# KTC-Security-Circle/3d-matching

Hardware: AMD Instinct MI355X
Metric: ICP iterations/sec + RANSAC hypotheses/sec, 100k↔100k pts, 1/2/4/8 GPU (higher is better)
Workload: dtype fp16-split MFMA NN screen + fp32 scan, exact fp64 NN decision, fp64 terms/solve; 1 GPU; cfg1: 100000<->100000 synthetic pair per GPU, 50 point-to-plane ICP iterations, brute-force NN (r=0.12), 1 GPU; ns=100000, nt_per_gpu=100000, parallelism=single, comm=none, comm_ranks=1

## Files before the change

### 3d-matching_amd/csrc/lds_dma.h

```cpp
#pragma once

#include <hip/hip_runtime.h>
#include <stdint.h>

namespace m3d {

__device__ __forceinline__ void lds_dma16(const void* src, void* wave_dst) {
  const uint32_t lds = __builtin_amdgcn_readfirstlane(
      (uint32_t)(uintptr_t)(__attribute__((address_space(3))) void*)wave_dst);
  uint32_t saved;
  asm volatile(
      "s_mov_b32 %0, m0\n\ts_mov_b32 m0, %2\n\ts_nop 0\n\tglobal_load_lds_dwordx4 %1, off\n\t"
      "s_mov_b32 m0, %0"
      : "=&s"(saved)
      : "v"(src), "s"(lds)
      : "memory");
}

__device__ __forceinline__ void lds_dma_wait() { asm volatile("s_waitcnt vmcnt(0)" ::: "memory"); }

}
```

### 3d-matching_amd/csrc/nn_brute.hip

```cpp
#include <algorithm>

#include "lds_dma.h"
#include "m3d_internal.h"
#include "nnkey.h"

#ifndef M3D_NN_BRUTE_PLAN_TU
#define M3D_NN_BRUTE_PLAN_TU 0
#endif
#ifndef M3D_NN_CLOCK
#define M3D_NN_CLOCK 0
#endif
#define M3D_NN_TU_MAIN (!M3D_NN_BRUTE_PLAN_TU)
#define M3D_NN_TU_PLAN_KERNEL (M3D_NN_BRUTE_PLAN_TU ? !M3D_NN_CLOCK : M3D_NN_CLOCK)
#if M3D_NN_TU_MAIN || M3D_NN_TU_PLAN_KERNEL

namespace m3d {

typedef _Float16 half8 __attribute__((ext_vector_type(8)));
typedef float floatx16 __attribute__((ext_vector_type(16)));

constexpr int kMG = 2;
constexpr int kMTile = 256;
constexpr int kTH = 4;
constexpr int kMTilePad = 1024;
constexpr int kMBlock = 512;
constexpr int kMQueries = (kMBlock / 64) * kMG * 32;

__device__ __forceinline__ void split16(float x, _Float16& hi, _Float16& lo) {
  hi = (_Float16)x;
  lo = (_Float16)(x - (float)hi);
}

union H8 {
  uint4 u;
  half8 h;
};

__device__ __forceinline__ uint32_t or16(const floatx16& k) {
  const auto b = [&](int i) { return __float_as_uint(k[i]); };
  const uint32_t o0 = __builtin_amdgcn_bitop3_b32(b(0), b(1), b(2), 0xFE);
  const uint32_t o1 = __builtin_amdgcn_bitop3_b32(b(3), b(4), b(5), 0xFE);
  const uint32_t o2 = __builtin_amdgcn_bitop3_b32(b(6), b(7), b(8), 0xFE);
  const uint32_t o3 = __builtin_amdgcn_bitop3_b32(b(9), b(10), b(11), 0xFE);
  const uint32_t o4 = __builtin_amdgcn_bitop3_b32(b(12), b(13), b(14), 0xFE);
  const uint32_t o5 = __builtin_amdgcn_bitop3_b32(o0, o1, o2, 0xFE);
  const uint32_t o6 = __builtin_amdgcn_bitop3_b32(o3, o4, b(15), 0xFE);
  return o5 | o6;
}

__device__ __forceinline__ void thr_operand(half8& b, float thr0, bool& force) {
  const float extra = 1.05f * ((32.0f * 1.01f * 5.9604645e-08f + 2.3841858e-07f) * fabsf(thr0) +
                               5.9604645e-08f);
  float thr = thr0 + extra;
  force = thr > 32768.0f;
  thr = fminf(fmaxf(thr, -32768.0f), 32768.0f);
  const _Float16 th = (_Float16)thr;
  const _Float16 tl = (_Float16)(thr - (float)th);
  b[3] = -th;
  b[4] = -tl;
}

#if M3D_NN_TU_MAIN
#ifndef M3D_NN_TILE_MORTON
#define M3D_NN_TILE_MORTON 1
#endif
__global__ __launch_bounds__(256) void pack16_sorted_kernel(const float4* __restrict__ sorted,
                                                            const int32_t* __restrict__ perm,
                                                            const float4* __restrict__ xyz32,
                                                            int64_t n, int64_t n_pad, float S,
                                                            uint4* __restrict__ mf16,
                                                            float4* __restrict__ mf32) {
  const int64_t k = (int64_t)blockIdx.x * 256 + threadIdx.x;
  if (k >= n_pad) return;
  H8 a, b;
  a.u = make_uint4(0, 0, 0, 0);
  b.u = make_uint4(0, 0, 0, 0);
  if (k < n) {
    const int32_t idx = __float_as_int(sorted[perm != nullptr ? perm[k] : k].w);
    const float4 t = xyz32[idx];
    _Float16 xh, xl, yh, yl, zh, zl, wh, wl;
    split16(t.x * S, xh, xl);
    split16(t.y * S, yh, yl);
    split16(t.z * S, zh, zl);
    split16(t.w * (S * S), wh, wl);
    a.h = half8{xh, xh, xl, yh, yh, yl, zh, zh};
    b.h = half8{zl, wh, wl, (_Float16)1, (_Float16)1, (_Float16)0, (_Float16)0, (_Float16)0};
    mf32[k] = make_float4(t.x, t.y, t.z, __int_as_float(idx));
  } else {
    b.h[1] = (_Float16)65504.0f;
    b.h[3] = (_Float16)1;
    b.h[4] = (_Float16)1;
    mf32[k] = make_float4(1.0e18f, 1.0e18f, 1.0e18f, __int_as_float(-1));
  }
  mf16[k] = a.u;
  mf16[n_pad + k] = b.u;
}

__global__ __launch_bounds__(kMTile) void tile_box_kernel(const float4* __restrict__ mf32,
                                                          float4* __restrict__ box) {
  const float4 t = mf32[(int64_t)blockIdx.x * kMTile + threadIdx.x];
  const bool real = __float_as_int(t.w) >= 0;
  float v[6] = {real ? t.x : kInf,  real ? t.y : kInf,  real ? t.z : kInf,
                real ? t.x : -kInf, real ? t.y : -kInf, real ? t.z : -kInf};
#pragma unroll
  for (int o = 1; o < 64; o <<= 1)
#pragma unroll
    for (int k = 0; k < 6; ++k) {
      const float w = __shfl_xor(v[k], o);
      v[k] = k < 3 ? fminf(v[k], w) : fmaxf(v[k], w);
    }
  __shared__ float part[kMTile / 64][6];
  if ((threadIdx.x & 63) == 0)
#pragma unroll
    for (int k = 0; k < 6; ++k) part[threadIdx.x >> 6][k] = v[k];
  __syncthreads();
  if (threadIdx.x != 0) return;
#pragma unroll
  for (int w = 1; w < kMTile / 64; ++w)
#pragma unroll
    for (int k = 0; k < 6; ++k) v[k] = k < 3 ? fminf(v[k], part[w][k]) : fmaxf(v[k], part[w][k]);
  box[2 * (int64_t)blockIdx.x] = make_float4(v[0], v[1], v[2], 0.0f);
  box[2 * (int64_t)blockIdx.x + 1] = make_float4(v[3], v[4], v[5], 0.0f);
}

hipError_t build_mfma_tiles(const m3d_cloud* c, Grid* g, TmpArena* ta, hipStream_t st) {
  const int64_t n = c->n;
  const int64_t n_pad = std::max<int64_t>((n + kMTilePad - 1) / kMTilePad * kMTilePad, kMTilePad);
  const int32_t* perm = nullptr;
  hipError_t e = M3D_NN_TILE_MORTON ? grid_morton_perm(g, ta, st, &perm) : hipSuccess;
  if (e != hipSuccess) return e;
  e = block_alloc(reinterpret_cast<void**>(&g->mf16), sizeof(uint4) * 2 * n_pad, st);
  if (e == hipSuccess) e = block_alloc(reinterpret_cast<void**>(&g->mf32), sizeof(float4) * n_pad, st);
  if (e == hipSuccess)
    e = block_alloc(reinterpret_cast<void**>(&g->mfbox), sizeof(float4) * 2 * (n_pad / kMTile), st);
  if (e != hipSuccess) {
    block_release(g->mf16);
    block_release(g->mf32);
    block_release(g->mfbox);
    g->mf16 = nullptr;
    g->mf32 = nullptr;
    g->mfbox = nullptr;
    return e;
  }
  g->mf_npad = n_pad;
  pack16_sorted_kernel<<<(unsigned)((n_pad + 255) / 256), 256, 0, st>>>(
      g->pts, perm, c->xyz32, n, n_pad, (float)c->s16, g->mf16, g->mf32);
  tile_box_kernel<<<(unsigned)(n_pad / kMTile), kMTile, 0, st>>>(g->mf32, g->mfbox);
  return hipGetLastError();
}

#endif

struct SeedArgs {
  const int32_t* prev;
  const float4* tgt;
  int64_t nt;
  int on;
};

__device__ __forceinline__ float4 seed_rec_prev(const SeedArgs& sa, int64_t i, int64_t off) {
  const int64_t j = sa.prev[i];
  float4 r = make_float4(0.0f, 0.0f, 0.0f, __int_as_float(-1));
  if (j >= off && j < off + sa.nt) {
    r = sa.tgt[j - off];
    r.w = __int_as_float((int32_t)j);
  }
  return r;
}

struct NnSlice {
  unsigned x, y, S;
};
struct NnPlan {
  const uint32_t* table;
  uint32_t* cnt;
  int nq, S;
};

__device__ __forceinline__ bool publish_k1(const SeedArgs& sa, unsigned y, uint64_t k1, bool changed) {
  return changed || (sa.on && y == 0 && key_real(k1));
}

__device__ void nn_slice_scan(const float4* __restrict__ src32, int64_t ns, const float4* __restrict__ tgt32,
                              int64_t jb, int64_t je, int64_t off, const IcpState* __restrict__ s,
                              int64_t* __restrict__ keys, uint32_t* __restrict__ near2,
                              const SeedArgs& sa, int64_t q0, unsigned bsx, unsigned bsy) {
  const float* Rt = s->Rt32;
  const float r2_hi = s->r2_hi;
  for (int qs = threadIdx.x; qs < kMQueries; qs += kMBlock) {
    const int64_t slot = q0 + (int64_t)bsx * kMQueries + qs;
    if (slot >= ns) return;
    const int64_t i = slot;
    float qx, qy, qz;
    const float4 p = src32[i];
    xform32(Rt, p, qx, qy, qz);
    const int64_t key = sa.on == 0 ? keys[i]
                                   : seed_key_rec(s, sa.on == 2 ? sa.tgt[i] : seed_rec_prev(sa, i, off), qx, qy, qz);
    uint64_t k1 = key == kKeyNone ? make_key(r2_hi, 0xFFFFFFFFu) : (uint64_t)key;
    float k1d = key_real_d2(k1), n2 = kInf;
    const uint64_t k10 = k1;
    for (int64_t j = jb; j < je; ++j) {
      const float4 t = tgt32[j];
      if (__float_as_int(t.w) < 0) continue;
      const float d2 = d2f(qx, qy, qz, t.x, t.y, t.z);
      if (d2 <= r2_hi) near_push(k1, k1d, n2, make_key(d2, (uint32_t)(off + __float_as_int(t.w))), d2);
    }
    const bool pk = publish_k1(sa, bsy, k1, k1 != k10);
    if (pk || n2 < kInf) near_publish((unsigned long long*)&keys[i], &near2[i], k1, n2, pk);
  }
}

__device__ __forceinline__ void nn_push_rows(const float4 (&t)[16], int64_t off, float qx, float qy, float qz,
                                             float r2_hi, uint64_t& k1, float& k1d, float& n2) {
#pragma unroll
  for (int reg = 0; reg < 16; ++reg) {
    const float d2 = d2f(qx, qy, qz, t[reg].x, t[reg].y, t[reg].z);
    const uint64_t kc = make_key(d2, (uint32_t)(off + __float_as_int(t[reg].w)));
    if (d2 <= r2_hi) near_push(k1, k1d, n2, kc, d2);
  }
}

__device__ __forceinline__ void nn_exact_rows(const float4* __restrict__ rows, int64_t off, int h,
                                              float qx, float qy, float qz, float r2_hi,
                                              uint64_t& k1, float& k1d, float& n2) {
  float4 t[16];
#pragma unroll
  for (int reg = 0; reg < 16; ++reg) t[reg] = rows[(reg & 3) + 8 * (reg >> 2) + 4 * h];
  nn_push_rows(t, off, qx, qy, qz, r2_hi, k1, k1d, n2);
}

__device__ __forceinline__ uint64_t shfl_xor64(uint64_t v, int m) {
  const uint32_t lo = (uint32_t)__shfl_xor((int)(uint32_t)v, m);
  const uint32_t hi = (uint32_t)__shfl_xor((int)(uint32_t)(v >> 32), m);
  return ((uint64_t)hi << 32) | lo;
}

__device__ __forceinline__ uint32_t wave_or32(uint32_t v) {
  int x = (int)v;
  x |= __builtin_amdgcn_mov_dpp(x, 0xB1, 0xF, 0xF, false);
  x |= __builtin_amdgcn_mov_dpp(x, 0x4E, 0xF, 0xF, false);
  x |= xor4_dpp(x);
  x |= __builtin_amdgcn_mov_dpp(x, 0x128, 0xF, 0xF, false);
  return (uint32_t)(__builtin_amdgcn_readlane(x, 0) | __builtin_amdgcn_readlane(x, 16) |
                    __builtin_amdgcn_readlane(x, 32) | __builtin_amdgcn_readlane(x, 48));
}

template <bool kMax>
__device__ __forceinline__ float wave_minmax(float v) {
  const auto mm = [](float a, float b) { return kMax ? fmaxf(a, b) : fminf(a, b); };
  v = mm(v, __int_as_float(__builtin_amdgcn_mov_dpp(__float_as_int(v), 0xB1, 0xF, 0xF, false)));
  v = mm(v, __int_as_float(__builtin_amdgcn_mov_dpp(__float_as_int(v), 0x4E, 0xF, 0xF, false)));
  v = mm(v, __int_as_float(xor4_dpp(__float_as_int(v))));
  v = mm(v, __int_as_float(__builtin_amdgcn_mov_dpp(__float_as_int(v), 0x128, 0xF, 0xF, false)));
  const int x = __float_as_int(v);
  return mm(mm(__int_as_float(__builtin_amdgcn_readlane(x, 0)), __int_as_float(__builtin_amdgcn_readlane(x, 16))),
            mm(__int_as_float(__builtin_amdgcn_readlane(x, 32)), __int_as_float(__builtin_amdgcn_readlane(x, 48))));
}

#ifndef M3D_NN_CULL
#define M3D_NN_CULL 1
#endif
#ifndef M3D_NN_REACH
#define M3D_NN_REACH 1
#endif
#ifndef M3D_NN_ENTRY
#define M3D_NN_ENTRY 1
#endif
#ifndef M3D_NN_SEED_REC
#define M3D_NN_SEED_REC 1
#endif
#ifndef M3D_NN_DEFER_BATCH
#define M3D_NN_DEFER_BATCH 1
#endif
#ifndef M3D_NN_DEFER_FILTER
#define M3D_NN_DEFER_FILTER 1
#endif
#if M3D_NN_CLOCK
constexpr int kClkBlocks = 16384, kClkWords = 8;
__device__ unsigned long long g_nn_clock[kClkWords * kClkBlocks];
#endif
struct QBox {
  float lo[3], hi[3], X;
};
__device__ __forceinline__ bool box_out_of_reach(const QBox& q, const float4& tlo, const float4& thi) {
  const float gx = fmaxf(0.0f, fmaxf(q.lo[0] - thi.x, tlo.x - q.hi[0]));
  const float gy = fmaxf(0.0f, fmaxf(q.lo[1] - thi.y, tlo.y - q.hi[1]));
  const float gz = fmaxf(0.0f, fmaxf(q.lo[2] - thi.z, tlo.z - q.hi[2]));
  return d2f(gx, gy, gz, 0.0f, 0.0f, 0.0f) > q.X;
}
__device__ __forceinline__ bool point_out_of_reach(float qx, float qy, float qz, float X, const float (&lo)[3],
                                                   const float (&hi)[3]) {
  const float gx = fmaxf(0.0f, fmaxf(qx - hi[0], lo[0] - qx));
  const float gy = fmaxf(0.0f, fmaxf(qy - hi[1], lo[1] - qy));
  const float gz = fmaxf(0.0f, fmaxf(qz - hi[2], lo[2] - qz));
  return d2f(gx, gy, gz, 0.0f, 0.0f, 0.0f) > X;
}

constexpr int kTT = kTH * kMTile;
constexpr int kSub = kTT / 32;
constexpr uint64_t kGMask = (kSub == 64) ? ~0ull : ((1ull << kSub) - 1ull);
constexpr int kDefer = 16;
static_assert(kMBlock == 2 * kMTile, "one 16-B operand half per thread per half tile");
static_assert(kSub * kMG <= 64, "hit mask holds every (group, sub-tile)");
static_assert(kSub == 32, "one 32-bit hit record per group and tile");
static_assert(kMBlock / 64 == 8, "eight wave boxes, lanes ^1 ^2 ^4");

struct QState {
  float qx, qy, qz, qq;
  int64_t qi;
  uint64_t k1;
  float k1d, n2;
  half8 bq;
};

__device__ __forceinline__ uint64_t group_mask(uint32_t bits) {
  uint64_t m = 0;
#pragma unroll
  for (int g = 0; g < kMG; ++g)
    if ((bits >> g) & 1u) m |= kGMask << (g * kSub);
  return m;
}

__device__ __forceinline__ float load_query(QState& q, QBox& lq, int64_t slot, int h, float4 p, float4 rec,
                                            int64_t ns, const IcpState* __restrict__ s, const SeedArgs& sa,
                                            const int64_t* __restrict__ keys) {
  const float* Rt = s->Rt32;
  const float r2_hi = s->r2_hi, S = s->mfma_scale;
  const int64_t i = slot < ns ? slot : -1;
  q.qi = i;
  q.n2 = kInf;
  float X = -1.0f;
  if (i >= 0) {
    xform32(Rt, p, q.qx, q.qy, q.qz);
    const int64_t key = sa.on ? seed_key_rec(s, rec, q.qx, q.qy, q.qz) : keys[i];
    q.k1 = key == kKeyNone ? make_key(r2_hi, 0xFFFFFFFFu) : (uint64_t)key;
    X = search_bound(key_d2(q.k1), s->band_e, r2_hi);
    lq.lo[0] = fminf(lq.lo[0], q.qx);
    lq.lo[1] = fminf(lq.lo[1], q.qy);
    lq.lo[2] = fminf(lq.lo[2], q.qz);
    lq.hi[0] = fmaxf(lq.hi[0], q.qx);
    lq.hi[1] = fmaxf(lq.hi[1], q.qy);
    lq.hi[2] = fmaxf(lq.hi[2], q.qz);
    lq.X = fmaxf(lq.X, X);
  } else {
    q.qx = q.qy = q.qz = 0.0f;
    q.k1 = (uint64_t)kKeyNone;
  }
  q.k1d = key_real_d2(q.k1);
  q.qq = fmaf(q.qz, q.qz, fmaf(q.qy, q.qy, q.qx * q.qx));
  _Float16 ah, al, bh, bl, ch, cl;
  split16(-2.0f * S * q.qx, ah, al);
  split16(-2.0f * S * q.qy, bh, bl);
  split16(-2.0f * S * q.qz, ch, cl);
  const _Float16 one = (_Float16)1.0f, zero = (_Float16)0.0f;
  q.bq = h == 0 ? half8{ah, al, ah, bh, bl, bh, ch, cl} : half8{ch, one, one, zero, zero, zero, zero, zero};
  return X;
}

__device__ __forceinline__ bool refresh_threshold(QState& q, int h, float X, float eps, float S2) {
  bool fg;
  half8 bt = q.bq;
  thr_operand(bt, X < 0.0f ? -1.0f : ((X - q.qq) + eps) * S2, fg);
  if (h == 1) q.bq = bt;
  return fg;
}

__device__ __forceinline__ QBox reduce_boxes(const QBox& lq, float4 (&qbox)[kMBlock / 64][2], int lane, int wave) {
  float wlo[3], whi[3];
#pragma unroll
  for (int k = 0; k < 3; ++k) {
    wlo[k] = wave_minmax<false>(lq.lo[k]);
    whi[k] = wave_minmax<true>(lq.hi[k]);
  }
  const float wX = wave_minmax<true>(lq.X);
  if (lane == 0) {
    qbox[wave][0] = make_float4(wlo[0], wlo[1], wlo[2], wX);
    qbox[wave][1] = make_float4(whi[0], whi[1], whi[2], 0.0f);
  }
  __syncthreads();
  float4 lo = qbox[lane & 7][0], hi = qbox[lane & 7][1];
#pragma unroll
  for (int o = 1; o < 8; o <<= 1) {
    const auto x = [&](float v) { return __int_as_float(xor_lane(__float_as_int(v), o, kWave)); };
    lo = make_float4(fminf(lo.x, x(lo.x)), fminf(lo.y, x(lo.y)), fminf(lo.z, x(lo.z)), fmaxf(lo.w, x(lo.w)));
    hi = make_float4(fmaxf(hi.x, x(hi.x)), fmaxf(hi.y, x(hi.y)), fmaxf(hi.z, x(hi.z)), 0.0f);
  }
  const auto u = [](float v) { return __int_as_float(__builtin_amdgcn_readfirstlane(__float_as_int(v))); };
  return QBox{{u(lo.x), u(lo.y), u(lo.z)}, {u(hi.x), u(hi.y), u(hi.z)}, u(lo.w)};
}

struct ReachArgs {
  const QState (&q)[kMG];
  const uint32_t& act;
  float be, r2_hi;
  uint64_t (&slot)[2][kMBlock / 64];
  int wave;
};
struct TileCursor {
  const float4* tbox;
  const float4* wbox;
  QBox bx;
  int lane, ntile, ty;
  int tc;
  uint64_t mb, mw;
  int par = 0;

  __device__ __forceinline__ void cull_round(const ReachArgs& ra) {
    const int tl = tc + (lane >> 2) * ty;
    bool kb = tl < ntile, kw = kb;
    float4 tlo = make_float4(0.0f, 0.0f, 0.0f, 0.0f), thi = tlo;
    if (M3D_NN_CULL && kb) {
      const int64_t hb = (int64_t)tl * kTH + (lane & 3);
      tlo = tbox[2 * hb];
      thi = tbox[2 * hb + 1];
      const float4 l0 = wbox[0], u0 = wbox[1];
      const QBox wq{{l0.x, l0.y, l0.z}, {u0.x, u0.y, u0.z}, l0.w};
      kb = !box_out_of_reach(bx, tlo, thi);
      kw = !box_out_of_reach(wq, tlo, thi);
    }
    mb = __ballot(kb);
    mw = __ballot(kw);
#if M3D_NN_CULL && M3D_NN_REACH
    if (mb == 0) return;
    float X[kMG];
#pragma unroll
    for (int g = 0; g < kMG; ++g)
      X[g] = (ra.act >> g) & 1u ? search_bound(key_d2(ra.q[g].k1), ra.be, ra.r2_hi) : -1.0f;
    uint64_t keep = 0;
    for (uint64_t m = mw; m != 0; m &= m - 1) {
      const int b = __builtin_amdgcn_readfirstlane(__builtin_ctzll(m));
      const auto rl = [&](float v) { return __int_as_float(__builtin_amdgcn_readlane(__float_as_int(v), b)); };
      const float lo[3] = {rl(tlo.x), rl(tlo.y), rl(tlo.z)}, hi[3] = {rl(thi.x), rl(thi.y), rl(thi.z)};
      bool reach = false;
#pragma unroll
      for (int g = 0; g < kMG; ++g)
        reach |= ((ra.act >> g) & 1u) &&
                 !point_out_of_reach(ra.q[g].qx, ra.q[g].qy, ra.q[g].qz, X[g], lo, hi);
      if (__any(reach)) keep |= 1ull << b;
    }
    mw = keep;
    par ^= 1;
    if (lane == 0) ra.slot[par][ra.wave] = mw;
    __syncthreads();
    const uint64_t w = ra.slot[par][lane & 7];
    int wl = (int)(uint32_t)w, wh = (int)(uint32_t)(w >> 32);
#pragma unroll
    for (int o = 1; o < 8; o <<= 1) {
      wl |= xor_lane(wl, o, kWave);
      wh |= xor_lane(wh, o, kWave);
    }
    mb = ((uint64_t)(uint32_t)__builtin_amdgcn_readfirstlane(wh) << 32) |
         (uint32_t)__builtin_amdgcn_readfirstlane(wl);
#endif
  }
  __device__ __forceinline__ void next(int& t, uint32_t& hmask, const ReachArgs& ra) {
    for (;;) {
      if (mb != 0) {
        const int k = __builtin_ctzll(mb) >> 2;
        t = tc + k * ty;
        hmask = (uint32_t)(mw >> (4 * k)) & 15u;
        mb &= ~(15ull << (4 * k));
        return;
      }
      tc += 16 * ty;
      if (tc >= ntile) {
        t = ntile;
        hmask = 0;
        return;
      }
      cull_round(ra);
    }
  }
};

__device__ __forceinline__ void stage_tile(uint4 (&dst)[2][kTT], const uint4* __restrict__ tgt16,
                                           int64_t nt_pad, int t, bool dma) {
#pragma unroll
  for (int u = 0; u < kTH; ++u) {
    const int e = threadIdx.x + u * kMBlock;
    const uint4* src = tgt16 + (e / kTT) * nt_pad + (int64_t)t * kTT + e % kTT;
    if (dma)
      lds_dma16(src, &dst[e / kTT][(e % kTT) & ~63]);
    else
      dst[e / kTT][e % kTT] = *src;
  }
}

__device__ __forceinline__ void sweep_tile(uint32_t (&rec)[kMG], const uint4 (&t16)[2][2][kTT], int buf,
                                           int h, int c, uint32_t hmask, const QState (&q)[kMG],
                                           const floatx16& zacc) {
#pragma unroll
  for (int g = 0; g < kMG; ++g) rec[g] = 0;
  constexpr int kSteps = 8 * kMG;
#pragma unroll
  for (int half = 0; half < kTH; ++half) {
    if (!((hmask >> half) & 1u)) {
#pragma unroll
      for (int g = 0; g < kMG; ++g) rec[g] <<= 8;
      continue;
    }
    H8 av[8];
#pragma unroll
    for (int sub = 0; sub < 8; ++sub) av[sub].u = t16[buf][h][half * kMTile + sub * 32 + c];
    floatx16 kc = __builtin_amdgcn_mfma_f32_32x32x16_f16(av[0].h, q[0].bq, zacc, 0, 0, 0);
#pragma unroll
    for (int t = 0; t < kSteps; ++t) {
      floatx16 kn;
      if (t + 1 < kSteps)
        kn = __builtin_amdgcn_mfma_f32_32x32x16_f16(av[(t + 1) / kMG].h, q[(t + 1) % kMG].bq, zacc, 0, 0, 0);
      __builtin_amdgcn_sched_barrier(0);
      rec[t % kMG] = __builtin_amdgcn_alignbit(rec[t % kMG], or16(kc), 31);
      __builtin_amdgcn_sched_barrier(0);
      if (t + 1 < kSteps) kc = kn;
    }
  }
}

__device__ __forceinline__ uint64_t hit_mask(const uint32_t (&rec)[kMG], uint32_t hmask, uint64_t force64) {
  uint64_t hm = 0;
  uint32_t any = rec[0];
#pragma unroll
  for (int g = 1; g < kMG; ++g) any |= rec[g];
  if (__any(any != 0)) {
#pragma unroll
    for (int g = 0; g < kMG; ++g) hm |= (uint64_t)wave_or32(__builtin_bitreverse32(rec[g])) << (g * kSub);
  }
  uint32_t sm = 0;
#pragma unroll
  for (int half = 0; half < kTH; ++half)
    if ((hmask >> half) & 1u) sm |= 0xFFu << (8 * half);
  uint64_t fm = 0;
#pragma unroll
  for (int g = 0; g < kMG; ++g) fm |= (uint64_t)sm << (g * kSub);
  return hm | (force64 & fm);
}

__device__ __forceinline__ bool nn_exact_subtiles(uint64_t mg, const float4* __restrict__ tile, int64_t off,
                                                  int h, float r2_hi, QState& q) {
  const uint64_t kb = q.k1;
  while (mg != 0) {
    const int sub = __builtin_ctzll(mg);
    mg &= mg - 1;
    nn_exact_rows(tile + sub * 32, off, h, q.qx, q.qy, q.qz, r2_hi, q.k1, q.k1d, q.n2);
    const uint64_t o1 = shfl_xor64(q.k1, 32);
    const float on2 = __shfl_xor(q.n2, 32);
    near_merge(q.k1, q.k1d, q.n2, o1, on2);
  }
  return q.k1 != kb;
}

__device__ __forceinline__ uint32_t nn_defer_hits(const half8& a, const half8& bq, const floatx16& zacc) {
  const floatx16 v = __builtin_amdgcn_mfma_f32_32x32x16_f16(a, bq, zacc, 0, 0, 0);
  uint32_t m = 0;
#pragma unroll
  for (int reg = 15; reg >= 0; --reg) m = __builtin_amdgcn_alignbit(m, __float_as_uint(v[reg]), 31);
  return m;
}
__device__ __forceinline__ void nn_push_hits(uint32_t m, const float4* rows, int64_t off, int h, float qx,
                                             float qy, float qz, float r2_hi, uint64_t& k1, float& k1d,
                                             float& n2) {
  while (m != 0) {
    const int reg = __builtin_ctz(m);
    m &= m - 1;
    const float4 t = rows[(reg & 3) + 8 * (reg >> 2) + 4 * h];
    push_within(k1, k1d, n2, d2f(qx, qy, qz, t.x, t.y, t.z), r2_hi, (uint32_t)(off + __float_as_int(t.w)));
  }
}

template <bool kPlan>
__device__ __forceinline__ void nn_mfma_body(const float4* __restrict__ src32, int64_t ns,
                                             const uint4* __restrict__ tgt16, const float4* __restrict__ tgt32,
                                             const float4* __restrict__ tbox, int64_t nt_pad, int64_t off,
                                             const IcpState* __restrict__ s, int64_t* __restrict__ keys,
                                             uint32_t* __restrict__ near2, const SeedArgs& sa, int64_t q0,
                                             const NnPlan& pl) {
#if M3D_NN_ENTRY
  uint32_t e_tab = kPlanEmpty;
  if (kPlan && pl.table != nullptr) e_tab = pl.table[blockIdx.x];
  int32_t st_done = s->done, st_plan = s->plan_ok, st_mfma = s->mfma_ok;
  asm volatile("" : "+s"(st_done), "+s"(st_plan), "+s"(st_mfma), "+s"(e_tab));
  if (st_done) return;
#else
  if (s->done) return;
#endif
#if M3D_NN_CLOCK
  const unsigned long long clk0 = __builtin_amdgcn_s_memrealtime();
#endif
  NnSlice bs{0u, 0u, 0u};
  if (kPlan && pl.table != nullptr) {
#if M3D_NN_ENTRY
    if (st_plan) {
      const uint32_t e = e_tab;
#else
    if (s->plan_ok) {
      const uint32_t e = pl.table[blockIdx.x];
#endif
      if (e == kPlanEmpty) return;
      bs = NnSlice{plan_x(e), plan_y(e), plan_S(e)};
    } else {
      const unsigned y = blockIdx.x / (unsigned)pl.nq;
      if (y >= (unsigned)pl.S) return;
      bs = NnSlice{blockIdx.x - y * (unsigned)pl.nq, y, (unsigned)pl.S};
    }
  }
#if M3D_NN_ENTRY
  if (!st_mfma) {
#else
  if (!s->mfma_ok) {
#endif
    const int64_t tstep = (int64_t)(kPlan ? bs.S : gridDim.y) * kTT;
    for (int64_t t0 = (int64_t)(kPlan ? bs.y : blockIdx.y) * kTT; t0 < nt_pad; t0 += tstep)
      nn_slice_scan(src32, ns, tgt32, t0, min(nt_pad, t0 + kTT), off, s, keys, near2, sa, q0,
                    kPlan ? bs.x : blockIdx.x, kPlan ? bs.y : blockIdx.y);
    return;
  }
  __shared__ uint4 t16[2][2][kTT];
  __shared__ uint64_t dlist[kMBlock / 64][kDefer];
  __shared__ uint32_t dtile[kMBlock / 64][kDefer];
  __shared__ float4 qbox[kMBlock / 64][2];
  __shared__ uint64_t rslot[2][kMBlock / 64];
#if M3D_NN_CLOCK
  __shared__ uint32_t clk_slow, clk_ticket;
  __shared__ unsigned long long clk_exit;
  if (threadIdx.x == 0) {
    clk_slow = 0;
    clk_ticket = 0;
    clk_exit = 0;
  }
  uint32_t clk_halves = 0;
#endif
  uint32_t kept = 0;
  __shared__ uint32_t slice_xy;
  if (kPlan && threadIdx.x == 0) slice_xy = bs.x | (bs.y << 16);
  const int lane = threadIdx.x & 63, wave = threadIdx.x >> 6;
  const int c = lane & 31, h = lane >> 5;
  const float r2_hi = s->r2_hi, eps = s->screen_eps_m, S = s->mfma_scale, be = s->band_e;
  const float S2 = S * S;

  QState q[kMG];
  uint32_t act = 0;
  uint32_t force = 0;
  uint32_t chg = 0;
  QBox lq{{kInf, kInf, kInf}, {-kInf, -kInf, -kInf}, -1.0f};
  const int64_t slot0 = q0 + (kPlan ? (int64_t)bs.x : (int64_t)blockIdx.x) * kMQueries + wave * kMG * 32 + c;
  float4 qp[kMG], qr[kMG];
#pragma unroll
  for (int g = 0; g < kMG; ++g) {
    const int64_t slot = slot0 + g * 32;
    qp[g] = src32[slot < ns ? slot : 0];
    qr[g] = make_float4(0.0f, 0.0f, 0.0f, 0.0f);
  }
  if (sa.on == 2) {
#pragma unroll
    for (int g = 0; g < kMG; ++g) {
      const int64_t slot = slot0 + g * 32;
      qr[g] = sa.tgt[slot < ns ? slot : 0];
    }
  } else if (sa.on) {
#pragma unroll
    for (int g = 0; g < kMG; ++g) {
      const int64_t slot = slot0 + g * 32;
      qr[g] = seed_rec_prev(sa, slot < ns ? slot : 0, off);
    }
  }
#pragma unroll
  for (int g = 0; g < kMG; ++g) {
    const int64_t slot = slot0 + g * 32;
    const float X = load_query(q[g], lq, slot, h, qp[g], qr[g], ns, s, sa, keys);
    if (q[g].qi >= 0) act |= 1u << g;
    if (__any(refresh_threshold(q[g], h, X, eps, S2))) force |= 1u << g;
  }
  const floatx16 zacc = {0.0f, 0.0f, 0.0f, 0.0f, 0.0f, 0.0f, 0.0f, 0.0f,
                         0.0f, 0.0f, 0.0f, 0.0f, 0.0f, 0.0f, 0.0f, 0.0f};
  uint32_t dfr = 0;
#pragma unroll
  for (int g = 0; g < kMG; ++g)
    if (!((force >> g) & 1u) && __all(q[g].qi < 0 || key_real(q[g].k1))) dfr |= 1u << g;
  int dn = 0;
  uint64_t dmask = group_mask(dfr);
  dmask = ((uint64_t)(uint32_t)__builtin_amdgcn_readfirstlane((int)(dmask >> 32)) << 32) |
          (uint32_t)__builtin_amdgcn_readfirstlane((int)(uint32_t)dmask);

  const QBox bx = reduce_boxes(lq, qbox, lane, wave);
  const int ntile = (int)(nt_pad / kTT);
  const ReachArgs ra{q, act, be, r2_hi, rslot, wave};
  TileCursor cur{tbox, qbox[wave], bx, lane, ntile, (int)(kPlan ? bs.S : gridDim.y), (int)(kPlan ? bs.y : blockIdx.y), 0, 0};
  cur.cull_round(ra);
  int t0, t1;
  uint32_t h0, h1;
  cur.next(t0, h0, ra);
  if (t0 < ntile) stage_tile(t16[0], tgt16, nt_pad, t0, false);
  const uint64_t force64 = group_mask(force);
  __syncthreads();
#if M3D_NN_CLOCK
  const unsigned long long clk1 = __builtin_amdgcn_s_memrealtime();
#endif
  int tog = 0;
  for (; t0 < ntile; t0 = t1, h0 = h1) {
    const int buf = kPlan ? (int)(kept & 1u) : tog;
    const int64_t j0 = (int64_t)t0 * kTT;
    if (kPlan || M3D_NN_CLOCK) ++kept;
#if M3D_NN_CLOCK
    clk_halves += (uint32_t)__builtin_popcount(h0);
#endif
    cur.next(t1, h1, ra);
    if (t1 < ntile) stage_tile(t16[buf ^ 1], tgt16, nt_pad, t1, true);
    uint32_t rec[kMG];
    sweep_tile(rec, t16, buf, h, c, h0, q, zacc);
    uint64_t hm = hit_mask(rec, h0, force64);
    const uint64_t hd = hm & dmask;
    if (hd != 0 && dn < kDefer) {
      if (lane == 0) {
        dlist[wave][dn] = hd;
        dtile[wave][dn] = (uint32_t)j0;
      }
      ++dn;
      hm &= ~hd;
    }
#pragma unroll
    for (int g = 0; g < kMG; ++g) {
      const uint64_t mg = (hm >> (g * kSub)) & kGMask;
      if (mg == 0) continue;
      chg |= (uint32_t)nn_exact_subtiles(mg, tgt32 + j0, off, h, r2_hi, q[g]) << g;
      refresh_threshold(q[g], h, (act >> g) & 1u ? search_bound(key_d2(q[g].k1), be, r2_hi) : -1.0f, eps, S2);
    }
    lds_dma_wait();
    __syncthreads();
    if (!kPlan) tog ^= 1;
  }
#if M3D_NN_CLOCK
  const unsigned long long clk2 = __builtin_amdgcn_s_memrealtime();
  if (lane == 0) atomicMax(&clk_slow, clk_halves);
#endif
#if M3D_NN_DEFER_BATCH
  if (dn > 0) {
#if M3D_NN_DEFER_FILTER
    constexpr int kStash = 8;
#else
    constexpr int kStash = 16;
#endif
    static_assert(kStash * kMG <= 32, "a batch's group flags in one word");
    static_assert(sizeof(t16) >= sizeof(float4) * (kMBlock / 64) * kStash * 32, "a stash per wave");
    float4* const stash = reinterpret_cast<float4*>(&t16[0][0][0]) + wave * (kStash * 32);
    const auto uni = [](uint32_t v) { return (uint32_t)__builtin_amdgcn_readfirstlane((int)v); };
    int e = 0;
    uint64_t ent = dlist[wave][0];
    ent = ((uint64_t)uni((uint32_t)(ent >> 32)) << 32) | uni((uint32_t)ent);
    uint32_t base = uni(dtile[wave][0]);
    const auto subs = [](uint64_t m) {
      uint32_t u = 0;
#pragma unroll
      for (int g = 0; g < kMG; ++g) u |= (uint32_t)(m >> (g * kSub)) & (uint32_t)kGMask;
      return u;
    };
    uint32_t U = subs(ent);
    const auto pop = [&](uint32_t& row0, uint32_t& gs) {
      row0 = 0;
      gs = 0;
      while (U == 0) {
        if (e + 1 >= dn) return;
        ++e;
        ent = dlist[wave][e];
        ent = ((uint64_t)uni((uint32_t)(ent >> 32)) << 32) | uni((uint32_t)ent);
        base = uni(dtile[wave][e]);
        U = subs(ent);
      }
      const int sub = __builtin_ctz(U);
      U &= U - 1;
      row0 = base + (uint32_t)sub * 32u;
#pragma unroll
      for (int g = 0; g < kMG; ++g) gs |= (uint32_t)((ent >> (g * kSub + sub)) & 1u) << g;
    };
    uint64_t kb[kMG];
#pragma unroll
    for (int g = 0; g < kMG; ++g) kb[g] = q[g].k1;
    for (;;) {
      uint32_t gsel = 0;
      float4 ld[kStash / 2];
#if M3D_NN_DEFER_FILTER
      H8 av[kStash];
#endif
#pragma unroll
      for (int k = 0; k < kStash / 2; ++k) {
        uint32_t ra, ga, rb, gb;
        pop(ra, ga);
        pop(rb, gb);
        gsel |= (ga | (gb << kMG)) << (2 * kMG * k);
        ld[k] = make_float4(0.0f, 0.0f, 0.0f, 0.0f);
        if (h == 0 ? ga != 0 : gb != 0) ld[k] = tgt32[(int64_t)(h == 0 ? ra : rb) + c];
#if M3D_NN_DEFER_FILTER
        av[2 * k].u = tgt16[(int64_t)h * nt_pad + ra + c];
        av[2 * k + 1].u = tgt16[(int64_t)h * nt_pad + rb + c];
#endif
      }
#pragma unroll
      for (int k = 0; k < kStash / 2; ++k) stash[(2 * k + h) * 32 + c] = ld[k];
      __builtin_amdgcn_fence(__ATOMIC_RELEASE, "wavefront");
      __builtin_amdgcn_wave_barrier();
      __builtin_amdgcn_fence(__ATOMIC_ACQUIRE, "wavefront");
#if M3D_NN_DEFER_FILTER
#pragma unroll
      for (int sl = 0; sl < kStash; ++sl) {
        const uint32_t gs = (gsel >> (kMG * sl)) & ((1u << kMG) - 1u);
        if (gs == 0) break;
        uint32_t hit[kMG];
#pragma unroll
        for (int g = 0; g < kMG; ++g) hit[g] = (gs >> g) & 1u ? nn_defer_hits(av[sl].h, q[g].bq, zacc) : 0u;
#pragma unroll
        for (int g = 0; g < kMG; ++g)
          if ((gs >> g) & 1u)
            nn_push_hits(hit[g], stash + sl * 32, off, h, q[g].qx, q[g].qy, q[g].qz, r2_hi, q[g].k1, q[g].k1d,
                         q[g].n2);
      }
#else
#pragma unroll 1
      for (int sl = 0; sl < kStash; ++sl) {
        const uint32_t gs = (gsel >> (kMG * sl)) & ((1u << kMG) - 1u);
        if (gs == 0) break;
        float4 t[16];
#pragma unroll
        for (int reg = 0; reg < 16; ++reg) t[reg] = stash[sl * 32 + (reg & 3) + 8 * (reg >> 2) + 4 * h];
#pragma unroll
        for (int g = 0; g < kMG; ++g)
          if ((gs >> g) & 1u) nn_push_rows(t, off, q[g].qx, q[g].qy, q[g].qz, r2_hi, q[g].k1, q[g].k1d, q[g].n2);
      }
#endif
      if (U == 0 && e + 1 >= dn) break;
      __builtin_amdgcn_fence(__ATOMIC_RELEASE, "wavefront");
      __builtin_amdgcn_wave_barrier();
    }
#pragma unroll
    for (int g = 0; g < kMG; ++g) {
      const uint64_t o1 = shfl_xor64(q[g].k1, 32);
      const float on2 = __shfl_xor(q[g].n2, 32);
      near_merge(q[g].k1, q[g].k1d, q[g].n2, o1, on2);
      chg |= (uint32_t)(q[g].k1 != kb[g]) << g;
    }
  }
#else
  for (int e = 0; e < dn; ++e) {
    const uint64_t ent = dlist[wave][e];
    const float4* tile = tgt32 + (int64_t)dtile[wave][e];
#pragma unroll
    for (int g = 0; g < kMG; ++g)
      chg |= (uint32_t)nn_exact_subtiles((ent >> (g * kSub)) & kGMask, tile, off, h, r2_hi, q[g]) << g;
  }
#endif
#if M3D_NN_CLOCK
  const unsigned long long clk2b = __builtin_amdgcn_s_memrealtime();
#endif
  const uint32_t sxy = kPlan ? slice_xy : 0u;
  const int64_t sxl = (int64_t)(sxy & 0xFFFFu);
  const unsigned syl = sxy >> 16;
#define M3D_NN_SX (kPlan ? sxl : (int64_t)blockIdx.x)
#define M3D_NN_SY (kPlan ? syl : blockIdx.y)
#pragma unroll
  for (int g = 0; g < kMG; ++g) {
    if (h != 0 || q[g].qi < 0) continue;
#if (M3D_NN_CULL && M3D_NN_REACH) || M3D_NN_DEFER_BATCH
    int cq = c;
    asm volatile("" : "+v"(cq));
    const int64_t qi = q0 + M3D_NN_SX * kMQueries + (wave * kMG + g) * 32 + cq;
#else
    const int64_t qi = q[g].qi;
#endif
    const bool pk = publish_k1(sa, M3D_NN_SY, q[g].k1, (chg >> g) & 1u);
    if (pk || q[g].n2 < kInf) near_publish((unsigned long long*)&keys[qi], &near2[qi], q[g].k1, q[g].n2, pk);
  }
  if (kPlan && pl.cnt != nullptr && threadIdx.x == 0) atomicAdd(&pl.cnt[M3D_NN_SX], kept);
#if M3D_NN_CLOCK
  {
    const unsigned long long clk3 = __builtin_amdgcn_s_memrealtime();
    const int64_t blk = (int64_t)blockIdx.y * gridDim.x + blockIdx.x;
    if (lane == 0) {
      atomicMax(&clk_exit, clk3);
      if (atomicAdd(&clk_ticket, 1u) == kMBlock / 64 - 1 && blk < kClkBlocks) {
        unsigned long long* rec = g_nn_clock + kClkWords * blk;
        rec[0] = clk0;
        rec[1] = clk1;
        rec[2] = clk2;
        rec[3] = atomicMax(&clk_exit, 0ull);
        rec[4] = kept;
        rec[5] = atomicMax(&clk_slow, 0u);
        rec[6] = (unsigned long long)M3D_NN_SX | ((unsigned long long)M3D_NN_SY << 32) | ((unsigned long long)cur.ty << 48);
        rec[7] = clk2b;
      }
    }
  }
#endif
}

#undef M3D_NN_SX
#undef M3D_NN_SY
#define M3D_NN_KERNEL_ARGS                                                                            \
  const float4 *__restrict__ src32, int64_t ns, const uint4 *__restrict__ tgt16,                      \
      const float4 *__restrict__ tgt32, const float4 *__restrict__ tbox, int64_t nt_pad, int64_t off, \
      const IcpState *__restrict__ s, int64_t *__restrict__ keys, uint32_t *__restrict__ near2, SeedArgs sa, int64_t q0
#if M3D_NN_TU_MAIN
__global__ __launch_bounds__(kMBlock) __attribute__((amdgpu_waves_per_eu(4))) void nn_mfma_kernel(M3D_NN_KERNEL_ARGS) {
  nn_mfma_body<false>(src32, ns, tgt16, tgt32, tbox, nt_pad, off, s, keys, near2, sa, q0, NnPlan{nullptr, nullptr, 0, 0});
}
#endif
hipError_t launch_nn_plan_kernel(unsigned blocks, hipStream_t st, M3D_NN_KERNEL_ARGS, NnPlan pl);
int nn_plan_kernel_blocks_per_cu();
#if M3D_NN_TU_PLAN_KERNEL
__global__ __launch_bounds__(kMBlock) __attribute__((amdgpu_waves_per_eu(4))) void nn_mfma_plan_kernel(
    M3D_NN_KERNEL_ARGS, NnPlan pl) {
  nn_mfma_body<true>(src32, ns, tgt16, tgt32, tbox, nt_pad, off, s, keys, near2, sa, q0, pl);
}
hipError_t launch_nn_plan_kernel(unsigned blocks, hipStream_t st, M3D_NN_KERNEL_ARGS, NnPlan pl) {
  nn_mfma_plan_kernel<<<dim3(blocks), kMBlock, 0, st>>>(src32, ns, tgt16, tgt32, tbox, nt_pad, off, s, keys, near2, sa,
                                                        q0, pl);
  return hipGetLastError();
}
int nn_plan_kernel_blocks_per_cu() {
  int per = 0;
  if (hipOccupancyMaxActiveBlocksPerMultiprocessor(&per, nn_mfma_plan_kernel, kMBlock, 0) != hipSuccess) return 0;
  return per > 0 ? per : 1;
}
#endif
#undef M3D_NN_KERNEL_ARGS
#if M3D_NN_TU_MAIN

static int64_t nn_grid_y(int64_t bx, int64_t ntiles, int64_t slots, bool cull) {
  const auto clamped = [&](int64_t S) { return std::min(std::max<int64_t>(S, 1), ntiles); };
  const int64_t s0 = clamped((2048 + bx - 1) / bx);
  if (slots <= 0 || ntiles <= 1) {
    const int64_t per = (ntiles + s0 - 1) / s0;
    return (ntiles + per - 1) / per;
  }
  if (cull) return clamped(slots / bx);
  int64_t best = s0;
  double best_eff = 0.0;
  for (int64_t S = s0; S <= std::min(2 * s0, ntiles); ++S) {
    const int64_t blocks = bx * S, rounds = (blocks + slots - 1) / slots;
    const double eff = (double)blocks / (double)(rounds * slots);
    if (eff > best_eff + 1e-9) {
      best_eff = eff;
      best = S;
    }
  }
  return best;
}

#if M3D_NN_CLOCK
}
extern "C" int m3d_debug_nn_clock(unsigned long long* out, int n) {
  return hipMemcpyFromSymbol(out, HIP_SYMBOL(m3d::g_nn_clock), sizeof(unsigned long long) * (size_t)n) == hipSuccess ? 0 : -1;
}
namespace m3d {
#endif
static bool icp_nn_uses_mfma(const m3d_icp* s) {
  return s->tgrid != nullptr && s->tgrid->mf16 != nullptr;
}

bool icp_nn_range_ok(const m3d_icp* s) {
  if (s->params.nn_method == M3D_NN_GRID) return s->sgrid != nullptr && s->sgrid->mpts != nullptr;
  return icp_nn_uses_mfma(s);
}

hipError_t launch_icp_nn(const m3d_icp* s, int64_t off, bool self_seed, hipStream_t st, int64_t q0,
                         int64_t q1) {
  const int64_t ns = q1 < 0 ? s->src->n : q1;
  if (ns <= q0 || s->tgt->n == 0) return hipSuccess;
  const Grid* tg = s->tgrid;
  const int64_t tt = (int64_t)kTH * kMTile;
  if (!icp_nn_uses_mfma(s) || tg->mf_npad % tt != 0) return hipErrorInvalidValue;
  const int64_t slots = nn_resident_slots();
  const int64_t bx = (ns - q0 + kMQueries - 1) / kMQueries;
  const int64_t gy = nn_grid_y(bx, tg->mf_npad / tt, slots, M3D_NN_CULL != 0);
  const bool by_rec = M3D_NN_SEED_REC != 0 && self_seed && off == 0 && s->tgt->rec64 != nullptr && s->seed != nullptr;
  const SeedArgs sa{s->corr, by_rec ? s->seed : s->tgt->xyz32, s->tgt->n, by_rec ? 2 : self_seed ? 1 : 0};
  const bool planned = nn_plan_on() && s->nn_qblocks > 0 && q0 == 0 && ns == s->src->n && bx == s->nn_qblocks &&
                       bx * gy <= s->nn_budget;
  if (planned)
    return launch_nn_plan_kernel((unsigned)s->nn_budget, st, s->src->xyz32, ns, tg->mf16, tg->mf32, tg->mfbox,
                                 tg->mf_npad, off, s->state, s->keys, s->near2, sa, q0,
                                 NnPlan{s->nn_table, s->nn_cnt, (int)bx, (int)gy});
  nn_mfma_kernel<<<dim3((unsigned)bx, (unsigned)gy), kMBlock, 0, st>>>(
        s->src->xyz32, ns, tg->mf16, tg->mf32, tg->mfbox, tg->mf_npad, off, s->state, s->keys, s->near2, sa, q0);
  return hipGetLastError();
}

int64_t nn_resident_slots() {
  static const int64_t slots = [] {
    int dev = 0, per = 0;
    hipDeviceProp_t p;
    if (hipGetDevice(&dev) != hipSuccess || hipGetDeviceProperties(&p, dev) != hipSuccess) return (int64_t)0;
    if (hipOccupancyMaxActiveBlocksPerMultiprocessor(&per, nn_mfma_kernel, kMBlock, 0) != hipSuccess)
      return (int64_t)0;
    const int pp = nn_plan_kernel_blocks_per_cu();
    per = per > 0 ? per : 1;
    if (pp > 0 && pp < per) per = pp;
    return (int64_t)p.multiProcessorCount * per;
  }();
  return slots;
}

bool nn_plan_on() {
  static const bool on = [] {
    const char* e = getenv("M3D_NN_PLAN");
    return !(e && atoi(e) == 0);
  }();
  return on;
}

void nn_plan_shape(int64_t ns, int32_t* qblocks, int32_t* budget) {
  const int64_t slots = nn_resident_slots(), bx = (ns + kMQueries - 1) / kMQueries;
  const bool ok = M3D_NN_CULL != 0 && slots > 0 && bx >= 1 && bx < slots && bx <= kPlanMaxQ && slots <= 0xFFFF;
  *qblocks = ok ? (int32_t)bx : 0;
  *budget = ok ? (int32_t)slots : 0;
}

PlanArgs nn_plan_args(const m3d_icp* s) {
  PlanArgs pa;
  if (!nn_plan_on() || s->nn_qblocks <= 0 || s->tgrid == nullptr) return pa;
  pa.cnt = s->nn_cnt;
  pa.seen = s->nn_seen;
  pa.table = s->nn_table;
  pa.n = s->nn_qblocks;
  pa.budget = s->nn_budget;
  pa.cap = (int32_t)plan_cap(kPlanSmax, s->tgrid->mf_npad / ((int64_t)kTH * kMTile));
  return pa;
}

#endif

}
#endif
```

Before: 20550 ICP iter/s (100k src x 100k tgt per GPU).

## Pack surviving tile halves into dense LDS windows and deepen DMA prefetch

```diff
diff --git a/3d-matching_amd/csrc/lds_dma.h b/3d-matching_amd/csrc/lds_dma.h
--- a/3d-matching_amd/csrc/lds_dma.h
+++ b/3d-matching_amd/csrc/lds_dma.h
@@ -19,4 +19,14 @@
 
 __device__ __forceinline__ void lds_dma_wait() { asm volatile("s_waitcnt vmcnt(0)" ::: "memory"); }
 
+__device__ __forceinline__ void lds_dma_wait_older(uint32_t newer) {
+  switch (newer) {
+    case 0: asm volatile("s_waitcnt vmcnt(0)" ::: "memory"); break;
+    case 1: asm volatile("s_waitcnt vmcnt(1)" ::: "memory"); break;
+    case 2: asm volatile("s_waitcnt vmcnt(2)" ::: "memory"); break;
+    case 3: asm volatile("s_waitcnt vmcnt(3)" ::: "memory"); break;
+    default: asm volatile("s_waitcnt vmcnt(4)" ::: "memory"); break;
+  }
 }
+
+}
diff --git a/3d-matching_amd/csrc/nn_brute.hip b/3d-matching_amd/csrc/nn_brute.hip
--- a/3d-matching_amd/csrc/nn_brute.hip
+++ b/3d-matching_amd/csrc/nn_brute.hip
@@ -272,6 +272,9 @@
 #ifndef M3D_NN_DEFER_BATCH
 #define M3D_NN_DEFER_BATCH 1
 #endif
+#ifndef M3D_NN_PACK
+#define M3D_NN_PACK 1
+#endif
 #ifndef M3D_NN_DEFER_FILTER
 #define M3D_NN_DEFER_FILTER 1
 #endif
@@ -404,6 +407,9 @@
   int tc;
   uint64_t mb, mw;
   int par = 0;
+#if M3D_NN_CLOCK
+  uint32_t need = 0;
+#endif
 
   __device__ __forceinline__ void cull_round(const ReachArgs& ra) {
     const int tl = tc + (lane >> 2) * ty;
@@ -459,6 +465,9 @@
         const int k = __builtin_ctzll(mb) >> 2;
         t = tc + k * ty;
         hmask = (uint32_t)(mw >> (4 * k)) & 15u;
+#if M3D_NN_CLOCK
+        need += (uint32_t)__builtin_popcount((uint32_t)(mb >> (4 * k)) & 15u);
+#endif
         mb &= ~(15ull << (4 * k));
         return;
       }
@@ -471,7 +480,42 @@
       cull_round(ra);
     }
   }
+  __device__ __forceinline__ bool next_half(uint32_t& row, uint32_t& mine, uint32_t& kept, const ReachArgs& ra) {
+    for (;;) {
+      if (mb != 0) {
+        const int b = __builtin_ctzll(mb);
+        row = (uint32_t)(tc + (b >> 2) * ty) * (uint32_t)kTT + (uint32_t)(b & 3) * (uint32_t)kMTile;
+        mine = (uint32_t)(mw >> b) & 1u;
+        mb &= mb - 1;
+        if (((mb >> (b & ~3)) & 15ull) == 0) ++kept;
+#if M3D_NN_CLOCK
+        ++need;
+#endif
+        return true;
+      }
+      if (tc >= ntile) return false;
+      tc += 16 * ty;
+      if (tc >= ntile) return false;
+      cull_round(ra);
+    }
+  }
 };
+
+__device__ __forceinline__ uint32_t stage_window(TileCursor& cur, uint4 (&dst)[2][kTT], uint32_t (&wrow)[kTH],
+                                                 const uint4* __restrict__ tgt16, int64_t nt_pad, int wave,
+                                                 uint32_t& kept, const ReachArgs& ra) {
+  uint32_t w = 0;
+#pragma unroll 1
+  for (int n = 0; n < kTH; ++n) {
+    uint32_t row, mine;
+    if (!cur.next_half(row, mine, kept, ra)) break;
+    const uint4* src = tgt16 + ((wave >> 2) ? nt_pad : 0) + row + (threadIdx.x & (kMTile - 1));
+    lds_dma16(src, &dst[wave >> 2][n * kMTile + (wave & 3) * 64]);
+    if (threadIdx.x == 0) wrow[n] = row;
+    w += 0x100u | (mine << n);
+  }
+  return w;
+}
 
 __device__ __forceinline__ void stage_tile(uint4 (&dst)[2][kTT], const uint4* __restrict__ tgt16,
                                            int64_t nt_pad, int t, bool dma) {
@@ -542,6 +586,22 @@
     const int sub = __builtin_ctzll(mg);
     mg &= mg - 1;
     nn_exact_rows(tile + sub * 32, off, h, q.qx, q.qy, q.qz, r2_hi, q.k1, q.k1d, q.n2);
+    const uint64_t o1 = shfl_xor64(q.k1, 32);
+    const float on2 = __shfl_xor(q.n2, 32);
+    near_merge(q.k1, q.k1d, q.n2, o1, on2);
+  }
+  return q.k1 != kb;
+}
+
+__device__ __forceinline__ bool nn_exact_slots(uint64_t mg, const float4* __restrict__ tgt32,
+                                               const uint32_t (&wrow)[kTH], int64_t off, int h, float r2_hi,
+                                               QState& q) {
+  const uint64_t kb = q.k1;
+  while (mg != 0) {
+    const int sub = __builtin_ctzll(mg);
+    mg &= mg - 1;
+    const uint32_t row0 = (uint32_t)__builtin_amdgcn_readfirstlane((int)wrow[sub >> 3]) + (uint32_t)(sub & 7) * 32u;
+    nn_exact_rows(tgt32 + row0, off, h, q.qx, q.qy, q.qz, r2_hi, q.k1, q.k1d, q.n2);
     const uint64_t o1 = shfl_xor64(q.k1, 32);
     const float on2 = __shfl_xor(q.n2, 32);
     near_merge(q.k1, q.k1d, q.n2, o1, on2);
@@ -614,9 +674,11 @@
                     kPlan ? bs.x : blockIdx.x, kPlan ? bs.y : blockIdx.y);
     return;
   }
+  constexpr bool kPack = M3D_NN_PACK == 2 || (M3D_NN_PACK == 1 && !kPlan);
   __shared__ uint4 t16[2][2][kTT];
   __shared__ uint64_t dlist[kMBlock / 64][kDefer];
-  __shared__ uint32_t dtile[kMBlock / 64][kDefer];
+  __shared__ uint32_t dtile[kMBlock / 64][kDefer][kPack ? kTH : 1];
+  __shared__ uint32_t wrow[2][kTH];
   __shared__ float4 qbox[kMBlock / 64][2];
   __shared__ uint64_t rslot[2][kMBlock / 64];
 #if M3D_NN_CLOCK
@@ -686,47 +748,95 @@
   const ReachArgs ra{q, act, be, r2_hi, rslot, wave};
   TileCursor cur{tbox, qbox[wave], bx, lane, ntile, (int)(kPlan ? bs.S : gridDim.y), (int)(kPlan ? bs.y : blockIdx.y), 0, 0};
   cur.cull_round(ra);
-  int t0, t1;
-  uint32_t h0, h1;
-  cur.next(t0, h0, ra);
-  if (t0 < ntile) stage_tile(t16[0], tgt16, nt_pad, t0, false);
-  const uint64_t force64 = group_mask(force);
-  __syncthreads();
-#if M3D_NN_CLOCK
-  const unsigned long long clk1 = __builtin_amdgcn_s_memrealtime();
-#endif
-  int tog = 0;
-  for (; t0 < ntile; t0 = t1, h0 = h1) {
-    const int buf = kPlan ? (int)(kept & 1u) : tog;
-    const int64_t j0 = (int64_t)t0 * kTT;
-    if (kPlan || M3D_NN_CLOCK) ++kept;
-#if M3D_NN_CLOCK
-    clk_halves += (uint32_t)__builtin_popcount(h0);
-#endif
-    cur.next(t1, h1, ra);
-    if (t1 < ntile) stage_tile(t16[buf ^ 1], tgt16, nt_pad, t1, true);
-    uint32_t rec[kMG];
-    sweep_tile(rec, t16, buf, h, c, h0, q, zacc);
-    uint64_t hm = hit_mask(rec, h0, force64);
-    const uint64_t hd = hm & dmask;
-    if (hd != 0 && dn < kDefer) {
-      if (lane == 0) {
-        dlist[wave][dn] = hd;
-        dtile[wave][dn] = (uint32_t)j0;
-      }
-      ++dn;
-      hm &= ~hd;
-    }
-#pragma unroll
-    for (int g = 0; g < kMG; ++g) {
-      const uint64_t mg = (hm >> (g * kSub)) & kGMask;
-      if (mg == 0) continue;
-      chg |= (uint32_t)nn_exact_subtiles(mg, tgt32 + j0, off, h, r2_hi, q[g]) << g;
-      refresh_threshold(q[g], h, (act >> g) & 1u ? search_bound(key_d2(q[g].k1), be, r2_hi) : -1.0f, eps, S2);
-    }
-    lds_dma_wait();
+  uint64_t force64;
+#if M3D_NN_CLOCK
+  unsigned long long clk1;
+  uint32_t clk_rounds = 0;
+#endif
+  if constexpr (kPack) {
+    uint32_t w0 = stage_window(cur, t16[0], wrow[0], tgt16, nt_pad, wave, kept, ra);
+    uint32_t w1 = stage_window(cur, t16[1], wrow[1], tgt16, nt_pad, wave, kept, ra);
+    force64 = group_mask(force);
+    lds_dma_wait_older(w1 >> 8);
     __syncthreads();
-    if (!kPlan) tog ^= 1;
+#if M3D_NN_CLOCK
+    clk1 = __builtin_amdgcn_s_memrealtime();
+#endif
+    for (int buf = 0; w0 != 0; buf ^= 1) {
+      const uint32_t h0 = w0 & 15u;
+#if M3D_NN_CLOCK
+      clk_halves += (uint32_t)__builtin_popcount(h0);
+      ++clk_rounds;
+#endif
+      uint32_t rec[kMG];
+      sweep_tile(rec, t16, buf, h, c, h0, q, zacc);
+      uint64_t hm = hit_mask(rec, h0, force64);
+      const uint64_t hd = hm & dmask;
+      if (hd != 0 && dn < kDefer) {
+        if (lane == 0) {
+          dlist[wave][dn] = hd;
+#pragma unroll
+          for (int k = 0; k < kTH; ++k) dtile[wave][dn][k] = wrow[buf][k];
+        }
+        ++dn;
+        hm &= ~hd;
+      }
+#pragma unroll
+      for (int g = 0; g < kMG; ++g) {
+        const uint64_t mg = (hm >> (g * kSub)) & kGMask;
+        if (mg == 0) continue;
+        chg |= (uint32_t)nn_exact_slots(mg, tgt32, wrow[buf], off, h, r2_hi, q[g]) << g;
+        refresh_threshold(q[g], h, (act >> g) & 1u ? search_bound(key_d2(q[g].k1), be, r2_hi) : -1.0f, eps, S2);
+      }
+      lds_dma_wait();
+      __syncthreads();
+      w0 = w1;
+      w1 = stage_window(cur, t16[buf], wrow[buf], tgt16, nt_pad, wave, kept, ra);
+    }
+  } else {
+    int t0, t1;
+    uint32_t h0, h1;
+    cur.next(t0, h0, ra);
+    if (t0 < ntile) stage_tile(t16[0], tgt16, nt_pad, t0, false);
+    force64 = group_mask(force);
+    __syncthreads();
+#if M3D_NN_CLOCK
+    clk1 = __builtin_amdgcn_s_memrealtime();
+#endif
+    int tog = 0;
+    for (; t0 < ntile; t0 = t1, h0 = h1) {
+      const int buf = kPlan ? (int)(kept & 1u) : tog;
+      const int64_t j0 = (int64_t)t0 * kTT;
+      if (kPlan || M3D_NN_CLOCK) ++kept;
+#if M3D_NN_CLOCK
+      clk_halves += (uint32_t)__builtin_popcount(h0);
+      ++clk_rounds;
+#endif
+      cur.next(t1, h1, ra);
+      if (t1 < ntile) stage_tile(t16[buf ^ 1], tgt16, nt_pad, t1, true);
+      uint32_t rec[kMG];
+      sweep_tile(rec, t16, buf, h, c, h0, q, zacc);
+      uint64_t hm = hit_mask(rec, h0, force64);
+      const uint64_t hd = hm & dmask;
+      if (hd != 0 && dn < kDefer) {
+        if (lane == 0) {
+          dlist[wave][dn] = hd;
+          dtile[wave][dn][0] = (uint32_t)j0;
+        }
+        ++dn;
+        hm &= ~hd;
+      }
+#pragma unroll
+      for (int g = 0; g < kMG; ++g) {
+        const uint64_t mg = (hm >> (g * kSub)) & kGMask;
+        if (mg == 0) continue;
+        chg |= (uint32_t)nn_exact_subtiles(mg, tgt32 + j0, off, h, r2_hi, q[g]) << g;
+        refresh_threshold(q[g], h, (act >> g) & 1u ? search_bound(key_d2(q[g].k1), be, r2_hi) : -1.0f, eps, S2);
+      }
+      lds_dma_wait();
+      __syncthreads();
+      if (!kPlan) tog ^= 1;
+    }
   }
 #if M3D_NN_CLOCK
   const unsigned long long clk2 = __builtin_amdgcn_s_memrealtime();
@@ -746,7 +856,9 @@
     int e = 0;
     uint64_t ent = dlist[wave][0];
     ent = ((uint64_t)uni((uint32_t)(ent >> 32)) << 32) | uni((uint32_t)ent);
-    uint32_t base = uni(dtile[wave][0]);
+    uint32_t base[kPack ? kTH : 1];
+#pragma unroll
+    for (int k = 0; k < (kPack ? kTH : 1); ++k) base[k] = uni(dtile[wave][0][k]);
     const auto subs = [](uint64_t m) {
       uint32_t u = 0;
 #pragma unroll
@@ -762,12 +874,18 @@
         ++e;
         ent = dlist[wave][e];
         ent = ((uint64_t)uni((uint32_t)(ent >> 32)) << 32) | uni((uint32_t)ent);
-        base = uni(dtile[wave][e]);
+#pragma unroll
+        for (int k = 0; k < (kPack ? kTH : 1); ++k) base[k] = uni(dtile[wave][e][k]);
         U = subs(ent);
       }
       const int sub = __builtin_ctz(U);
       U &= U - 1;
-      row0 = base + (uint32_t)sub * 32u;
+      if constexpr (kPack) {
+        const int sl = sub >> 3;
+        row0 = (sl == 0 ? base[0] : sl == 1 ? base[1] : sl == 2 ? base[2] : base[kTH - 1]) + (uint32_t)(sub & 7) * 32u;
+      } else {
+        row0 = base[0] + (uint32_t)sub * 32u;
+      }
 #pragma unroll
       for (int g = 0; g < kMG; ++g) gs |= (uint32_t)((ent >> (g * kSub + sub)) & 1u) << g;
     };
@@ -840,10 +958,16 @@
 #else
   for (int e = 0; e < dn; ++e) {
     const uint64_t ent = dlist[wave][e];
-    const float4* tile = tgt32 + (int64_t)dtile[wave][e];
-#pragma unroll
-    for (int g = 0; g < kMG; ++g)
-      chg |= (uint32_t)nn_exact_subtiles((ent >> (g * kSub)) & kGMask, tile, off, h, r2_hi, q[g]) << g;
+    if constexpr (kPack) {
+#pragma unroll
+      for (int g = 0; g < kMG; ++g)
+        chg |= (uint32_t)nn_exact_slots((ent >> (g * kSub)) & kGMask, tgt32, dtile[wave][e], off, h, r2_hi, q[g]) << g;
+    } else {
+      const float4* tile = tgt32 + (int64_t)dtile[wave][e][0];
+#pragma unroll
+      for (int g = 0; g < kMG; ++g)
+        chg |= (uint32_t)nn_exact_subtiles((ent >> (g * kSub)) & kGMask, tile, off, h, r2_hi, q[g]) << g;
+    }
   }
 #endif
 #if M3D_NN_CLOCK
@@ -880,7 +1004,7 @@
         rec[1] = clk1;
         rec[2] = clk2;
         rec[3] = atomicMax(&clk_exit, 0ull);
-        rec[4] = kept;
+        rec[4] = kept | ((unsigned long long)cur.need << 16) | ((unsigned long long)clk_rounds << 32);
         rec[5] = atomicMax(&clk_slow, 0u);
         rec[6] = (unsigned long long)M3D_NN_SX | ((unsigned long long)M3D_NN_SY << 32) | ((unsigned long long)cur.ty << 48);
         rec[7] = clk2b;
```

Result: no change. 20420 ICP iter/s (100k src x 100k tgt per GPU) (-0.6%).
